# citiususc/veryfasttree

Hardware: AMD Instinct MI355X
Metric: profile-ops/sec (higher is better)
Workload: dtype f32; 1 GPU; c4_1M_x200_nt_tophits; n_seqs=1000000, n_pos=200, active_nodes=750000, top_k=2000

## Files before the change

### veryfasttree_amd/csrc/vft_api.hip

```cpp
#include <hip/hip_runtime.h>
#include <csignal>
#include <unistd.h>

#include <cmath>
#include <cstdarg>
#include <cstdio>
#include <cstdlib>
#include <cstring>
#include <new>
#include <algorithm>
#include <utility>
#include <vector>
#include <chrono>

#include "../../include/vft_hip.h"
#include "vft_owned.h"
#include "vft_staging.h"
#define VFT_PAIR_STAGE_CAP 2048
#include "vft_kernels_ml.h"

VFT_ML_HEAVY_INSTANCES(extern)
#include "vft_kernels_ml_long.h"
VFT_ML_LONG_INSTANCES(extern)
#include "vft_kernels_nj.h"
// ... 1915 lines not shown
    if (ids) {
        if (n <= 0) return VFT_OK;
        if (nActive > c->maxStamp) c->maxStamp = nActive;
        if (n == 1) {
            if (ids[0] < 0 || ids[0] >= c->maxnode) return fail(c, VFT_ERR_INVALID, "vft_out_distances: bad node");
            SweepArgs s{};
            s.nActive = nActive;
            s.totdiam = totdiam;
            s.force = 1;
            VFT_DISPATCH(c, launch((k_out_distance_one<REAL, NC>), dim3(1), dim3(VFT_WG), pw_lds_bytes(c) / c->pwWaves, c->stream,
                                   arena<REAL>(c), ids[0], s));
            LAUNCHCHK(c);
            return VFT_OK;
        }
        Stage st;
        if (int r = st.open(c, (size_t) n * 8, VFT_SMALL_BYTES)) return r;
        VFTCHK(st.put(0, ids, (size_t) n * 8));
        if (int r = launch_out_distances(c, st.dev<const int64_t>(0), n, nActive, 0, totdiam, true)) return r;
        return st.finish();
    }
    return launch_out_distances(c, nullptr, 0, nActive, 0, totdiam, true);
}

static void kernel_event(vft_ctx *c) {
    if (!c->timeKernels) return;
    if (c->kevUsed == c->kev.size()) {
        hipEvent_t e;
        if (hipEventCreate(&e) != hipSuccess) return;
        c->kev.push_back(e);
    }
    hipEventRecord(c->kev[c->kevUsed++], c->stream);
}

static int64_t slot_nodes(const vft_ctx *c, int slot) { return (c->d.nTiles + (slot ? 4 : 0)) * VFT_TILE; }

static int ensure_slots(vft_ctx *c, int count) {
    if (count > VFT_MAX_SLOTS) return fail(c, VFT_ERR_INVALID, "more than %d sweep slots", VFT_MAX_SLOTS);
    c->slots.reserve(VFT_MAX_SLOTS);
    const size_t rs = c->rs;
    bool added = false;
    while ((int) c->slots.size() < count) {
        const int slot = (int) c->slots.size();
        const size_t N = (size_t) slot_nodes(c, slot);
        c->slots.emplace_back();
        vft_ctx::SweepSlotHost &h = c->slots.back();
        const int r = own_group(c, [&]() -> int {
            void **reals[] = {&h.swDist, &h.swWeight, &h.swCrit};
            for (void **p: reals) OWNCHK(own_dev(c, p, N * rs, 0));
            const size_t nPartCap = (size_t) cdiv((int64_t) N, VFT_WG);
            OWNCHK(own_dev(c, &h.partMin, nPartCap * 8));
            OWNCHK(own_dev(c, &h.partMax, nPartCap * 8));
            OWNCHK(own_dev(c, &h.sel, sizeof(SelectState), 0));
            OWNCHK(own_dev(c, &h.slices, (size_t) VFT_NBINS * 4, 0));
            OWNCHK(own_dev(c, &h.candKey, (size_t) VFT_CAND_CAP * 8, 0));
            OWNCHK(own_dev(c, &h.candId, (size_t) VFT_CAND_CAP * 4, 0));
            const size_t resB = sizeof(SelectHeader) + (size_t) c->hitsCap * sizeof(vft_hit_f64);
            OWNCHK(own_dev(c, &h.dRes, resB));
            OWNCHK(own_host(c, &h.hRes, &h.hResDev, resB, sizeof(SelectHeader)));
            if (slot > 0 && c->cfg.n_codes == 4) {
                const size_t nPosPad = (size_t) c->d.nChunk * VFT_CHUNK;
                OWNCHK(own_dev(c, &h.qW, nPosPad * rs));
                OWNCHK(own_dev(c, &h.qF, nPosPad * 4 * rs));
                OWNCHK(own_dev(c, &h.qC, nPosPad));
                OWNCHK(own_dev(c, &h.qEnc, (size_t) c->d.nChunk * sizeof(uint4)));
                OWNCHK(own_dev(c, &h.qTab, nPosPad * 5 * sizeof(double2)));
            }
            return VFT_OK;
        });
        if (r) {
            c->slots.pop_back();
            return r;
        }
        added = true;
    }
    if (added) HIPCHK(c, hipDeviceSynchronize());
    return VFT_OK;
}

static int wait_headers(vft_ctx *c, int s0, int count, unsigned long long seq) {
    if (c->faultNoFlag) {
        seq += 1ull << 40;
        c->faultNoFlag = false;
    }
    auto raised = [&]() {
        for (int s = s0; s < s0 + count; s++)
            if ((unsigned long long) __atomic_load_n(&((const SelectHeader *) c->slots[(size_t) s].hRes)->pad2, __ATOMIC_ACQUIRE) != seq) return false;
        return true;
    };
    std::chrono::steady_clock::time_point t0;
    for (long spins = 0;; spins++) {
        if (raised()) return VFT_OK;
        if (spins == 200000) t0 = std::chrono::steady_clock::now();
        if (spins >= 200000 && (spins & 0xFFFF) == 0) {
            const hipError_t e = hipStreamQuery(c->stream);
            if (e == hipSuccess) {
                if (raised()) return VFT_OK;
                return fail(c, VFT_ERR_TIMEOUT, "the stream has drained but a selection never published its result");
            }
            if (e != hipErrorNotReady) return fail(c, VFT_ERR_HIP, "stream error while waiting: %s", hipGetErrorString(e));
            if (std::chrono::duration<double>(std::chrono::steady_clock::now() - t0).count() > c->waitLimitS)
                return fail(c, VFT_ERR_TIMEOUT, "no selection result after %.0f s (the stream is still busy)", c->waitLimitS);
        }
    }
}

template <typename REAL, typename HIT>
static int run_select(vft_ctx *c, int K, const int64_t *queries, int64_t lo, int64_t hi, int32_t k) {
    std::vector<SelSlot> hs((size_t) K);
    for (int s = 0; s < K; s++) {
        const vft_ctx::SweepSlotHost &h = c->slots[(size_t) s];
        SelSlot &d = hs[(size_t) s];
        d.crit = h.swCrit;
        d.dist = h.swDist;
        d.weight = h.swWeight;
        d.partMin = h.partMin;
        d.partMax = h.partMax;
        d.sel = h.sel;
        d.slices = h.slices;
        d.candKey = h.candKey;
        d.candId = h.candId;
        d.hits = h.dRes + sizeof(SelectHeader);
        d.hdr = (SelectHeader *) h.dRes;
        d.hostHdr = (SelectHeader *) h.hResDev;
        d.hostHits = h.hResDev + sizeof(SelectHeader);
        d.query = queries[s];
        d.nPart = h.nPart;
        d.pad = 0;
    }
    Stage st;
    if (int r = st.open(c, hs.size() * sizeof(SelSlot), Stage::RING_ONLY)) return r;
    st.put(0, hs.data(), hs.size() * sizeof(SelSlot));
    const SelSlot *slots = st.dev<const SelSlot>(0);
    auto round = [&](const SelSlot *sl, unsigned ny, int first, int s0) -> int {
        const unsigned long long seq = ++c->signalSeq;
        launch((k_select_hist<REAL>), dim3(VFT_SEL_WGS, ny), dim3(VFT_WG), 0, c->stream, sl, lo, hi, first);
        launch((k_select_collect<REAL>), dim3(VFT_SEL_WGS, ny), dim3(VFT_WG), 0, c->stream, sl, lo, hi, (unsigned int) k);
        launch((k_select_rank<REAL, HIT>), dim3(VFT_CAND_CAP * VFT_RANK_LANES / VFT_WG, ny), dim3(VFT_WG), 0, c->stream, sl, k, lo, hi, (long long) seq);
        LAUNCHCHK(c);
        return wait_headers(c, s0, (int) ny, seq);
    };
    if (int r = round(slots, (unsigned) K, 1, 0)) return r;
    for (int s = 0; s < K; s++) {
        const SelectHeader *h = (const SelectHeader *) c->slots[(size_t) s].hRes;
        for (int level = 0; h->overflow; level++) {
            if (level == VFT_MAX_LEVEL)
                return fail(c, VFT_ERR_STATE, "top-k select: more than %d hits tied at the k-th criterion", VFT_CAND_CAP);
            launch(k_select_refine, dim3(1, 1), dim3(1), 0, c->stream, slots + s);
            if (int r = round(slots + s, 1u, 0, s)) return r;
        }
    }
    return VFT_OK;
}

static int sweep_one(vft_ctx *c, int slot, int64_t query, int64_t nActive, int64_t nDiffAllow, double totdiam, bool staged = false) {
    if (int r = flush_pending(c)) return r;
    const int64_t lo = c->shardLo, hi = c->shardHi < c->maxnode ? c->shardHi : c->maxnode;
    if (c->maxStamp - nActive > nDiffAllow)
        if (int r = launch_out_distances(c, nullptr, 0, nActive, nDiffAllow, totdiam, false)) return r;
    if ((int64_t) c->hNOut[query] - nActive > nDiffAllow) {
        if (nActive > c->maxStamp) c->maxStamp = nActive;
        SweepArgs s{};
        s.nActive = nActive;
        s.nDiffAllow = nDiffAllow;
        s.totdiam = totdiam;
        s.force = 0;
        VFT_DISPATCH(c, launch((k_out_distance_one<REAL, NC>), dim3(1), dim3(VFT_WG), pw_lds_bytes(c) / c->pwWaves, c->stream,
                               arena<REAL>(c), query, s));
        LAUNCHCHK(c);
    }
    SweepArgs s{};
    s.query = query;
    s.lo = lo;
    s.hi = hi;
    s.nActive = nActive;
    s.nDiffAllow = nDiffAllow;
    s.totdiam = totdiam;
    s.queryIsLeaf = query < c->d.nSeqs ? 1 : 0;
#ifdef VFT_ABLATE
    if (const char *dbg = getenv("VFT_SWEEP_ABLATE")) s.pad = atoi(dbg);
#endif
    const int64_t span = hi > lo ? hi - lo : 0;
    const bool ntPath = c->cfg.n_codes == 4 && !c->hasDm;
    const unsigned grid = ntPath ? sweep_nt_grid(c, s, !s.queryIsLeaf) : cdiv(span > 0 ? span : 1, VFT_WG);
    c->slots[(size_t) slot].nPart = (int) grid;
    const int64_t nPosPad = (int64_t) c->d.nChunk * VFT_CHUNK;
    if (c->cfg.n_codes == 4 && !c->hasDm) {
        if (c->cfg.precision == 4) {
            const QueryBuf<float> Q = staged ? qbuf_slot<float>(c, slot) : qbuf<float>(c, 0);
            if (!staged) launch((k_extract_query<float, 4>), dim3(cdiv(nPosPad, 256)), dim3(256), 0, c->stream, arena<float>(c), query, Q);
            if (s.queryIsLeaf) launch_sweep_nt<float, MODE_CRIT_LEAFQ>(c, s, grid, Q, true, slot);
            else launch_sweep_nt<float, MODE_CRIT>(c, s, grid, Q, true, slot);
        } else {
            const QueryBuf<double> Q = staged ? qbuf_slot<double>(c, slot) : qbuf<double>(c, 0);
            if (!staged) launch((k_extract_query<double, 4>), dim3(cdiv(nPosPad, 256)), dim3(256), 0, c->stream, arena<double>(c), query, Q);
            if (s.queryIsLeaf) launch_sweep_nt<double, MODE_CRIT_LEAFQ>(c, s, grid, Q, true, slot);
            else launch_sweep_nt<double, MODE_CRIT>(c, s, grid, Q, true, slot);
        }
    } else {
        kernel_event(c);
        if (c->cfg.n_codes == 20 && c->hasDm && c->aaLds && span > 0) {
            const unsigned g = c->cfg.precision == 4 ? launch_sweep_aa<float, MODE_CRIT>(c, s, 0, slot) : launch_sweep_aa<double, MODE_CRIT>(c, s, 0, slot);
            c->slots[(size_t) slot].nPart = (int) g;
        } else if (span <= 32768) {
            const unsigned wgrid = (unsigned) std::min<int64_t>(cdiv(span > 0 ? span : 1, c->pwWaves), 256 * 16);
            c->slots[(size_t) slot].nPart = (int) wgrid;
            VFT_DISPATCH(c, (launch((k_sweep_wave<REAL, NC>), dim3(wgrid), dim3(64 * c->pwWaves), pw_lds_bytes(c), c->stream,
                                    arena<REAL>(c), s, sweepout<REAL>(c, slot))));
        } else {
            VFT_DISPATCH(c, (launch((k_sweep_generic<REAL, NC>), dim3(grid), dim3(VFT_WG), 0, c->stream,
                                    arena<REAL>(c), s, sweepout<REAL>(c, slot))));
        }
        kernel_event(c);
        kernel_event(c);
    }
    LAUNCHCHK(c);
    return VFT_OK;
}

template <typename REAL, int S>
static int sweep_group(vft_ctx *c, bool leafSeeds, const int *slotOf, const int64_t *queries, int64_t nActive, int64_t nDiffAllow, double totdiam, const void *mq, const void *lq) {
    SweepArgs s{};
    s.query = queries[slotOf[0]];
    s.lo = c->shardLo;
    s.hi = c->shardHi < c->maxnode ? c->shardHi : c->maxnode;
    s.nActive = nActive;
    s.nDiffAllow = nDiffAllow;
    s.totdiam = totdiam;
    s.queryIsLeaf = leafSeeds ? 1 : 0;
    const unsigned grid = sweep_nt_grid(c, s, !leafSeeds);
    MultiLeafQ<REAL, S> M;
    for (int q = 0; q < S; q++) {
        M.Q[q] = qbuf_slot<REAL>(c, slotOf[q]);
        M.O[q] = sweepout<REAL>(c, slotOf[q]);
        M.query[q] = queries[slotOf[q]];
        c->slots[(size_t) slotOf[q]].nPart = (int) grid;
    }
    M.mq = (const REAL *) mq;
    M.lq = (const uint32_t *) lq;
    kernel_event(c);
    if (grid && leafSeeds) launch((k_sweep_nt_leafq_multi<REAL, S>), dim3(grid), dim3(VFT_WG), 0, c->stream, arena<REAL>(c), M, s);
    if (grid && !leafSeeds) launch((k_sweep_nt_profq_multi<REAL, S>), dim3(grid), dim3(VFT_WG), 0, c->stream, arena<REAL>(c), M, s);
    kernel_event(c);
    kernel_event(c);
    if (c->timeKernels) c->kevSweeps += S - 1;
    LAUNCHCHK(c);
    return VFT_OK;
}

static bool mixed_sweep_fits(vft_ctx *c) {
    SweepArgs s{};
    s.lo = c->shardLo;
    s.hi = c->shardHi < c->maxnode ? c->shardHi : c->maxnode;
    const unsigned grid = sweep_nt_grid(c, s, true);
    if (!s.nLeafWG || grid == (unsigned) s.nLeafWG || s.hi <= s.leafEnd) return false;
    if (c->rs != 4) return false;
    const int64_t N = slot_nodes(c, 1);
    return (int64_t) cdiv(s.leafEnd - s.lo, VFT_WG) + (int64_t) (grid - (unsigned) s.nLeafWG) <= (int64_t) cdiv(N, VFT_WG);
}

template <typename REAL>
static int sweep_mixed(vft_ctx *c, const int *leafPos, const int *profPos, const int64_t *queries, int64_t nActive, int64_t nDiffAllow, double totdiam, const void *mq, const void *lq) {
    constexpr int S = 4;
    MixedArgs<REAL, S, S> a;
    memset((void *) &a, 0, sizeof(a));
    a.A = arena<REAL>(c);
    SweepArgs &s = a.s;
    s.query = queries[profPos[0]];
    s.lo = c->shardLo;
    s.hi = c->shardHi < c->maxnode ? c->shardHi : c->maxnode;
    s.nActive = nActive;
    s.nDiffAllow = nDiffAllow;
    s.totdiam = totdiam;
    s.queryIsLeaf = 0;
    const unsigned gridP = sweep_nt_grid(c, s, true);
    a.nInt = (int32_t) (gridP - (unsigned) s.nLeafWG);
    a.nLeafHeavy = (int32_t) cdiv(s.leafEnd - s.lo, VFT_WG);
    for (int q = 0; q < S; q++) {
        a.M.L.Q[q] = qbuf_slot<REAL>(c, leafPos[q]);
        a.M.L.O[q] = sweepout<REAL>(c, leafPos[q]);
        a.M.L.query[q] = queries[leafPos[q]];
        c->slots[(size_t) leafPos[q]].nPart = a.nLeafHeavy + a.nInt;
        a.M.P.Q[q] = qbuf_slot<REAL>(c, profPos[q]);
        a.M.P.O[q] = sweepout<REAL>(c, profPos[q]);
        a.M.P.query[q] = queries[profPos[q]];
        c->slots[(size_t) profPos[q]].nPart = (int) gridP;
    }
    a.M.L.mq = nullptr;
    a.M.L.lq = (const uint32_t *) lq;
    a.M.P.mq = (const REAL *) mq;
    a.M.P.lq = nullptr;
    kernel_event(c);
    launch((k_sweep_nt_mixed_multi<REAL, S, S>), dim3((unsigned) (a.nInt + a.nLeafHeavy + s.nLeafWG)), dim3(VFT_WG), 0, c->stream, a);
    kernel_event(c);
    kernel_event(c);
    if (c->timeKernels) c->kevSweeps += 2 * S - 1;
    LAUNCHCHK(c);
    return VFT_OK;
}

static int no_slot(vft_ctx *c) { return fail(c, VFT_ERR_STATE, "the context has no sweep buffers (vft_create failed)"); }

static int sweep_args_ok(vft_ctx *c, int64_t query, int64_t nActive, int32_t k) {
    if (c->slots.empty()) return no_slot(c);
    if (!c->leavesUp) return fail(c, VFT_ERR_STATE, "vft_sweep before vft_upload_leaves");
    if (query < 0 || query >= c->maxnode || nActive < 3 || k < 0 || k > c->hitsCap)
        return fail(c, VFT_ERR_INVALID, "vft_sweep: bad arguments (query %lld, nActive %lld, k %d)", (long long) query,
// ... 2045 lines not shown
```

### veryfasttree_amd/csrc/vft_kernels_nj.h

```cpp
#pragma once
#include "vft_device.h"

#define VFT_WG 256

template <typename REAL>
struct QueryBuf {
    REAL *w;
    uint8_t *code;
    REAL *f;
    uint4 *enc;
    double2 *tab;
};

template <typename REAL>
__device__ __forceinline__ void vft_query_tab(const QueryBuf<REAL> &q, int64_t p, REAL wq, const REAL *f) {
#pragma unroll
    for (int c = 0; c < 5; c++) {
        double2 v = make_double2(0.0, 0.0);
        if (c < 4 && wq > 0) {
            const double wgt = (double) wq;
            const double piece = 1.0 - (double) f[c < 4 ? c : 0];
            v = make_double2(wgt * piece, wgt);
        }
        q.tab[p * 5 + c] = v;
// ... 1896 lines not shown
        const REAL dd = A.diameter[i] + A.diameter[j];
        d = d - dd;
    }
    dist[t] = d;
}

#define VFT_PB_A 8
template <typename REAL, int NC>
__global__ __launch_bounds__(VFT_WG) void k_pairs_block_tiled(Arena<REAL> A, const int64_t *idsA, int64_t nA, const int64_t *idsB,
                                                              int64_t nB, REAL *dist) {
    extern __shared__ __attribute__((aligned(16))) double pbLds[];
    const int64_t nPos = A.d.nPos;
    REAL *sF = (REAL *) pbLds;
    REAL *sWt = sF + (int64_t) VFT_PB_A * nPos * NC;
    int32_t *sCode = (int32_t *) (sWt + (int64_t) VFT_PB_A * nPos);
    const int64_t a0 = (int64_t) blockIdx.y * VFT_PB_A;
    for (int64_t e = threadIdx.x; e < (int64_t) VFT_PB_A * nPos; e += VFT_WG) {
        const int64_t a = e / nPos, p = e % nPos;
        const int64_t id = a0 + a < nA ? idsA[a0 + a] : -1;
        Col<REAL, NC> c;
        c.w = 0;
        c.code = VFT_NOCODE_;
        c.vec = false;
#pragma unroll
        for (int k = 0; k < NC; k++) c.f[k] = 0;
        if (id >= 0) vft_load_col_ml<REAL, NC>(A, id, p, c);
        sWt[e] = c.w;
        sCode[e] = c.code | (c.vec ? 256 : 0);
#pragma unroll
        for (int k = 0; k < NC; k++) sF[e * NC + k] = c.vec ? c.f[k] : (REAL) 0;
    }
    __syncthreads();
    const int64_t b = (int64_t) blockIdx.x * VFT_WG + threadIdx.x;
    const int64_t jb = b < nB ? idsB[b] : -1;
    if (jb < 0) return;
    double top[VFT_PB_A], den[VFT_PB_A];
#pragma unroll
    for (int a = 0; a < VFT_PB_A; a++) top[a] = den[a] = 0.0;
    for (int64_t p = 0; p < nPos; p++) {
        Col<REAL, NC> cb;
        vft_load_col_ml<REAL, NC>(A, jb, p, cb);
        if (!(cb.w > 0)) continue;
#pragma unroll
        for (int a = 0; a < VFT_PB_A; a++) {
            const int64_t e = (int64_t) a * nPos + p;
            Col<REAL, NC> ca;
            ca.w = sWt[e];
            if (!(ca.w > 0)) continue;
            const int32_t cc = sCode[e];
            ca.code = cc & 255;
            ca.vec = (cc & 256) != 0;
#pragma unroll
            for (int k = 0; k < NC; k++) ca.f[k] = sF[e * NC + k];
            const REAL ww = ca.w * cb.w;
            const double wgt = (double) ww;
            den[a] += wgt;
            top[a] += wgt * vft_piece<REAL, NC>(A, ca, cb, nullptr);
        }
    }
#pragma unroll
    for (int a = 0; a < VFT_PB_A; a++) {
        if (a0 + a >= nA) break;
        const int64_t i = idsA[a0 + a];
        if (i < 0 || i == jb) continue;
        REAL d = (REAL) (den[a] > 0 ? top[a] / den[a] : 1.0);
        if (!(i < A.d.nSeqs && jb < A.d.nSeqs)) {
            const REAL dd = A.diameter[i] + A.diameter[jb];
            d = d - dd;
        }
        dist[(a0 + a) * nB + b] = d;
    }
}

template <typename REAL, int NC, bool WGPAIR>
__global__ __launch_bounds__(VFT_WG) void k_refresh_list(Arena<REAL> A, const int64_t *ids, int64_t n, int64_t nForced, SweepArgs s) {
    extern __shared__ __attribute__((aligned(16))) double pwLds[];
    const int64_t t = WGPAIR ? (int64_t) blockIdx.x : (int64_t) blockIdx.x * VFT_PW_WAVES + (threadIdx.x >> 6);
    if (t >= n) return;
    const int64_t v = ids[t];
    if (t < nForced ? (int64_t) A.nOutActive[v] == s.nActive : !((int64_t) A.nOutActive[v] - s.nActive > s.nDiffAllow)) return;
    REAL d, w;
    if (WGPAIR) vft_pair_block<REAL, NC>(A, v, -1, true, pwLds, pwLds + A.d.nPosPad, d, w);
    else vft_pair_wave<REAL, NC>(A, v, -1, true, vft_pw_lds(pwLds, A.d.nPosPad, 0), vft_pw_lds(pwLds, A.d.nPosPad, 1), d, w);
    if ((WGPAIR ? threadIdx.x : (threadIdx.x & 63)) != 0) return;
    const REAL od = vft_out_distance<REAL>(d, w, s.nActive, A.selfweight[v], A.selfdist[v], A.diameter[v], s.totdiam);
    A.outDist[v] = od;
    A.mOutDist[v] = od;
    A.mNOut[v] = (int32_t) s.nActive;
    A.nOutActive[v] = (int32_t) s.nActive;
}

#define VFT_LB_A 16
template <typename REAL>
__global__ __launch_bounds__(VFT_WG) void k_leaf_block(Arena<REAL> A, const int64_t *idsA, int64_t nA, const int64_t *idsB,
                                                       int64_t nB, SweepArgs s, REAL *dist, REAL *weight, REAL *crit) {
    const int lane = threadIdx.x & 63, wave = __builtin_amdgcn_readfirstlane((int) (threadIdx.x >> 6));
    const int64_t tb = (int64_t) blockIdx.x * 64 + lane;
    const int64_t a0 = (int64_t) blockIdx.y * 64 + (int64_t) wave * VFT_LB_A;
    if (a0 >= nA) return;
    const int64_t b = tb < nB ? idsB[tb] : -1;
    const bool bOk = b >= 0 && b < A.d.nSeqs;
    const uint4 *bT = A.leafT + vft_leaf_idx(A.d, bOk ? b >> 6 : 0, 0, (int) (bOk ? b & 63 : 0));
    int64_t aId[VFT_LB_A];
    const uint4 *aT[VFT_LB_A];
#pragma unroll
    for (int u = 0; u < VFT_LB_A; u++) {
        int64_t a = a0 + u < nA ? idsA[a0 + u] : -1;
        if (a < 0 || a >= A.d.nSeqs) a = -1;
        aId[u] = a;
        aT[u] = A.leafT + vft_leaf_idx(A.d, a >= 0 ? a >> 6 : 0, 0, (int) (a >= 0 ? a & 63 : 0));
    }
    int nUse[VFT_LB_A], nSame[VFT_LB_A];
#pragma unroll
    for (int u = 0; u < VFT_LB_A; u++) nUse[u] = nSame[u] = 0;
    const int nChunk = A.d.nChunk;
    for (int c = 0; c < nChunk; c++) {
        const uint4 vb = bT[(int64_t) c * VFT_TILE];
#pragma unroll
        for (int u = 0; u < VFT_LB_A; u++) {
            typedef const __attribute__((address_space(4))) vft_u4_t *sp_t;
            const vft_u4_t q = *(sp_t) (aT[u] + (int64_t) c * VFT_TILE);
            uint4 va;
            va.x = q.x; va.y = q.y; va.z = q.z; va.w = q.w;
            vft_seq_counts(va, vb, nUse[u], nSame[u]);
        }
    }
    if (tb >= nB) return;
    const REAL outB = bOk ? A.outDist[b] : (REAL) 0;
    const int64_t nOutB = bOk ? A.nOutActive[b] : s.nActive;
#pragma unroll
    for (int u = 0; u < VFT_LB_A; u++) {
        if (a0 + u >= nA) break;
        const int64_t a = aId[u];
        REAL d = (REAL) 1e20, w = 0, cr = (REAL) 1e20;
        if (a >= 0 && bOk) {
            w = (REAL) (double) nUse[u];
            d = (REAL) (nUse[u] > 0 ? (double) (nUse[u] - nSame[u]) / (double) nUse[u] : 1.0);
            cr = vft_criterion<REAL>(d, A.outDist[a], A.nOutActive[a], outB, nOutB, s.nActive);
        }
        const int64_t o = (a0 + u) * nB + tb;
        dist[o] = d;
        weight[o] = w;
        crit[o] = cr;
    }
}

#define VFT_NBINS 1024
#define VFT_DIGIT_BITS 10
#define VFT_VK_FRAC_BITS 40
#define VFT_MAX_LEVEL 4
#define VFT_SEL_WGS 128
#define VFT_CAND_CAP 8192

struct SelectState {
    double lo, scale;
    unsigned long long prefix;
    unsigned int level;
    unsigned int threshBin;
    unsigned int nCand;
    unsigned int overflow;
    unsigned int nBelow;
    unsigned int nThresh;
    unsigned int nIn;
    unsigned int rankDone;
};

struct SelectHeader;
struct SelSlot {
    const void *crit, *dist, *weight;
    const void *partMin, *partMax;
    SelectState *sel;
    unsigned int *slices;
    uint64_t *candKey;
    int32_t *candId;
    void *hits;
    SelectHeader *hdr, *hostHdr;
    void *hostHits;
    int64_t query;
    int32_t nPart, pad;
};

__device__ __forceinline__ unsigned long long vft_vk(double x, double lo, double scale) {
    const double y = (x - lo) * scale;
    const double top = 1125899906842623.0;
    return y <= 0.0 ? 0ull : (y >= top ? (unsigned long long) top : (unsigned long long) y);
}
__device__ __forceinline__ unsigned int vft_level_shift(unsigned int level) {
    return (unsigned int) (VFT_VK_FRAC_BITS - VFT_DIGIT_BITS * (int) level);
}

__global__ void k_select_refine(const SelSlot *slots) {
    SelectState *S = slots[blockIdx.y].sel;
    S->nIn += S->nBelow;
    S->prefix = (S->prefix << VFT_DIGIT_BITS) | S->threshBin;
    S->level += 1;
    S->nCand = 0;
    S->overflow = 0;
    S->rankDone = 0;
}

template <typename REAL>
__global__ __launch_bounds__(VFT_WG) void k_select_hist(const SelSlot *slots, int64_t lo, int64_t hi, int first) {
    const SelSlot &sl = slots[blockIdx.y];
    const REAL *crit = (const REAL *) sl.crit;
    SelectState *S = sl.sel;
    unsigned int *slices = sl.slices;
    __shared__ unsigned int lh4[4][VFT_NBINS];
    unsigned int *lh = lh4[threadIdx.x & 3];
    __shared__ double smin[VFT_WG / 64], smax[VFT_WG / 64];
    for (int t = threadIdx.x; t < 4 * VFT_NBINS; t += VFT_WG) lh4[0][t] = 0;
    double vlo, scale;
    unsigned long long prefix;
    unsigned int level;
    if (first) {
        const REAL *partMin = (const REAL *) sl.partMin, *partMax = (const REAL *) sl.partMax;
        double cmin = 1e30, cmax = -1e30;
        for (int t = threadIdx.x; t < sl.nPart; t += VFT_WG) {
            const double a = (double) partMin[t], b = (double) partMax[t];
            cmin = a < cmin ? a : cmin;
            cmax = b > cmax ? b : cmax;
        }
#pragma unroll
        for (int off = 32; off > 0; off >>= 1) {
            const double a = __shfl_xor(cmin, off, 64), b = __shfl_xor(cmax, off, 64);
            cmin = a < cmin ? a : cmin;
            cmax = b > cmax ? b : cmax;
        }
        if ((threadIdx.x & 63) == 0) {
            smin[threadIdx.x >> 6] = cmin;
            smax[threadIdx.x >> 6] = cmax;
        }
        __syncthreads();
        cmin = smin[0];
        cmax = smax[0];
#pragma unroll
        for (int w = 1; w < VFT_WG / 64; w++) {
            cmin = smin[w] < cmin ? smin[w] : cmin;
            cmax = smax[w] > cmax ? smax[w] : cmax;
        }
        const double span = cmax > cmin ? cmax - cmin : 1.0;
        vlo = cmin;
        scale = 1023.9990234375 * 1099511627776.0 / span;
        prefix = 0;
        level = 0;
        if (blockIdx.x == 0 && threadIdx.x == 0) {
            S->lo = vlo;
            S->scale = scale;
            S->prefix = 0;
            S->level = 0;
            S->nCand = 0;
            S->overflow = 0;
            S->nIn = 0;
            S->rankDone = 0;
        }
    } else {
        __syncthreads();
        vlo = S->lo;
        scale = S->scale;
        prefix = S->prefix;
        level = S->level;
    }
    const unsigned int shift = vft_level_shift(level);
    const int64_t stride = (int64_t) gridDim.x * VFT_WG;
    int64_t j = lo + (int64_t) blockIdx.x * VFT_WG + threadIdx.x;
    for (; j + 3 * stride < hi; j += 4 * stride) {
        REAL c[4];
#pragma unroll
        for (int u = 0; u < 4; u++) c[u] = crit[j + u * stride];
#pragma unroll
        for (int u = 0; u < 4; u++) {
            if (c[u] < (REAL) 1e20) {
                const unsigned long long vk = vft_vk((double) c[u], vlo, scale);
                if ((vk >> (shift + VFT_DIGIT_BITS)) == prefix) atomicAdd(&lh[(vk >> shift) & (VFT_NBINS - 1)], 1u);
            }
        }
    }
    for (; j < hi; j += stride) {
        const REAL c = crit[j];
        if (c < (REAL) 1e20) {
            const unsigned long long vk = vft_vk((double) c, vlo, scale);
            if ((vk >> (shift + VFT_DIGIT_BITS)) == prefix) atomicAdd(&lh[(vk >> shift) & (VFT_NBINS - 1)], 1u);
        }
    }
    __syncthreads();
    for (int t = threadIdx.x; t < VFT_NBINS; t += VFT_WG) {
        const unsigned int v = lh4[0][t] + lh4[1][t] + lh4[2][t] + lh4[3][t];
        if (v) atomicAdd(&slices[t], v);
    }
}

template <typename REAL>
__global__ __launch_bounds__(VFT_WG) void k_select_collect(const SelSlot *slots, int64_t lo, int64_t hi, unsigned int k) {
    const SelSlot &sl = slots[blockIdx.y];
    const REAL *crit = (const REAL *) sl.crit;
    SelectState *S = sl.sel;
    uint64_t *candKey = sl.candKey;
    int32_t *candId = sl.candId;
    __shared__ unsigned int lcount, lbase;
    __shared__ uint64_t lkey[VFT_CAND_CAP / 8];
    __shared__ int32_t lid[VFT_CAND_CAP / 8];
    if (threadIdx.x == 0) lcount = 0;
    __shared__ unsigned int wsum[VFT_WG / 64], sTb, sBelow, sThresh;
    unsigned int tb;
    {
        constexpr int PER = VFT_NBINS / VFT_WG;
        const unsigned int *gh = sl.slices;
        const int lane = threadIdx.x & 63, wave = threadIdx.x >> 6;
        unsigned int v[PER], mine = 0;
#pragma unroll
        for (int u = 0; u < PER; u++) {
            v[u] = gh[threadIdx.x * PER + u];
            mine += v[u];
        }
        unsigned int incl = mine;
#pragma unroll
        for (int off = 1; off < 64; off <<= 1) {
            const unsigned int o = __shfl_up(incl, off, 64);
            if (lane >= off) incl += o;
        }
        if (lane == 63) wsum[wave] = incl;
        if (threadIdx.x == 0) {
            sTb = VFT_NBINS;
            sBelow = 0;
            sThresh = 0;
        }
        __syncthreads();
        unsigned int before = incl - mine, total = 0;
#pragma unroll
        for (int w = 0; w < VFT_WG / 64; w++) {
            if (w < wave) before += wsum[w];
            total += wsum[w];
        }
        unsigned int need = k > S->nIn ? k - S->nIn : 0;
        if (need > total) need = total;
        if (need > 0 && before < need && before + mine >= need) {
            unsigned int b = before;
#pragma unroll
            for (int u = 0; u < PER; u++) {
                if (b < need && b + v[u] >= need) {
                    sTb = (unsigned int) (threadIdx.x * PER + u);
                    sBelow = b;
                    sThresh = v[u];
                }
                b += v[u];
            }
        }
        __syncthreads();
        tb = sTb;
        if (blockIdx.x == 0 && threadIdx.x == 0) {
            S->threshBin = tb;
            S->nBelow = sBelow;
            S->nThresh = sThresh;
        }
    }
    const double vlo = S->lo, scale = S->scale;
    const unsigned long long prefix = S->prefix;
    const unsigned int shift = vft_level_shift(S->level);
    const int64_t stride = (int64_t) gridDim.x * VFT_WG;
    auto take = [&](int64_t j, REAL c) {
        if (!(c < (REAL) 1e20)) return;
        const unsigned long long vk = vft_vk((double) c, vlo, scale);
        const unsigned long long up = vk >> (shift + VFT_DIGIT_BITS);
        if (up < prefix || (up == prefix && tb < VFT_NBINS && ((vk >> shift) & (VFT_NBINS - 1)) <= tb)) {
            const unsigned int slot = atomicAdd(&lcount, 1u);
            if (slot < VFT_CAND_CAP / 8) {
                lkey[slot] = sizeof(REAL) == 4 ? (uint64_t) vft_order_f32((float) c) : vft_order_f64((double) c);
                lid[slot] = (int32_t) j;
            }
        }
    };
    int64_t j = lo + (int64_t) blockIdx.x * VFT_WG + threadIdx.x;
    for (; j + 3 * stride < hi; j += 4 * stride) {
        REAL c[4];
#pragma unroll
        for (int u = 0; u < 4; u++) c[u] = crit[j + u * stride];
#pragma unroll
        for (int u = 0; u < 4; u++) take(j + u * stride, c[u]);
    }
    for (; j < hi; j += stride) take(j, crit[j]);
    __syncthreads();
    const unsigned int n = lcount;
    if (n > VFT_CAND_CAP / 8) {
        if (threadIdx.x == 0) S->overflow = 1;
        return;
    }
    if (threadIdx.x == 0) lbase = n ? atomicAdd(&S->nCand, n) : 0;
    __syncthreads();
    const unsigned int base = lbase;
    if (base + n > VFT_CAND_CAP) {
        if (threadIdx.x == 0) S->overflow = 1;
        return;
    }
    for (unsigned int t = threadIdx.x; t < n; t += VFT_WG) {
        candKey[base + t] = lkey[t];
        candId[base + t] = lid[t];
    }
}

struct SelectHeader {
    unsigned int nCand, overflow, shift, pad;
    long long bestJ;
    long long pad2;
};

template <typename HIT>
__device__ __forceinline__ void vft_hit_publish(HIT *dst, const HIT &h) {
    static_assert(sizeof(HIT) % 8 == 0, "hit records are whole 8-byte words");
    unsigned long long w[sizeof(HIT) / 8];
    __builtin_memcpy(w, &h, sizeof(HIT));
#pragma unroll
    for (unsigned int t = 0; t < sizeof(HIT) / 8; t++)
        __hip_atomic_store((unsigned long long *) dst + t, w[t], __ATOMIC_RELAXED, __HIP_MEMORY_SCOPE_AGENT);
}
template <typename HIT>
__device__ __forceinline__ HIT vft_hit_fetch(const HIT *src) {
    unsigned long long w[sizeof(HIT) / 8];
#pragma unroll
    for (unsigned int t = 0; t < sizeof(HIT) / 8; t++)
        w[t] = __hip_atomic_load((const unsigned long long *) src + t, __ATOMIC_RELAXED, __HIP_MEMORY_SCOPE_AGENT);
    HIT h;
    __builtin_memcpy(&h, w, sizeof(HIT));
    return h;
}

#define VFT_RANK_TILE 2048
#define VFT_RANK_LANES 16
template <typename REAL, typename HIT>
__global__ __launch_bounds__(VFT_WG) void k_select_rank(const SelSlot *slots, int32_t k, int64_t lo, int64_t hi, long long seq) {
    const SelSlot &sl = slots[blockIdx.y];
    SelectState *S = sl.sel;
    const uint64_t *candKey = sl.candKey;
    const int32_t *candId = sl.candId;
    const REAL *dist = (const REAL *) sl.dist, *weight = (const REAL *) sl.weight, *crit = (const REAL *) sl.crit;
    HIT *hits = (HIT *) sl.hits;
    HIT *hostHits = (HIT *) sl.hostHits;
    __shared__ uint64_t sk[VFT_RANK_TILE];
    __shared__ int32_t si[VFT_RANK_TILE];
    const unsigned int n = S->overflow ? 0u : (S->nCand < VFT_CAND_CAP ? S->nCand : VFT_CAND_CAP);
    const unsigned int perWg = VFT_WG / VFT_RANK_LANES;
    const unsigned int span = n > (unsigned int) k ? n : (unsigned int) k;
    if (blockIdx.x * perWg >= span) return;
    const unsigned int cand = blockIdx.x * perWg + threadIdx.x / VFT_RANK_LANES;
    const unsigned int sub = threadIdx.x % VFT_RANK_LANES;
    const bool mine = cand < n;
    const uint64_t myKey = mine ? candKey[cand] : 0;
    const int32_t myId = mine ? candId[cand] : 0;
    unsigned int rank = 0;
    for (unsigned int base = 0; base < n; base += VFT_RANK_TILE) {
        __syncthreads();
        for (unsigned int u = threadIdx.x; u < VFT_RANK_TILE; u += VFT_WG) {
            sk[u] = base + u < n ? candKey[base + u] : ~0ull;
            si[u] = base + u < n ? candId[base + u] : -1;
        }
        __syncthreads();
        const unsigned int lim = n - base < VFT_RANK_TILE ? n - base : VFT_RANK_TILE;
        if (mine) {
#pragma unroll 8
            for (unsigned int u = sub; u < lim; u += VFT_RANK_LANES) {
                const uint64_t ku = sk[u];
                const int32_t iu = si[u];
                rank += (ku < myKey || (ku == myKey && iu > myId)) ? 1u : 0u;
            }
        }
    }
#pragma unroll
    for (int off = VFT_RANK_LANES / 2; off > 0; off >>= 1) rank += __shfl_xor(rank, off, VFT_RANK_LANES);
    if (sub == 0) {
        if (mine && rank < (unsigned int) k) {
            HIT h;
            h.j = myId;
            h.dist = dist[myId];
            h.weight = weight[myId];
            h.criterion = crit[myId];
            vft_hit_publish<HIT>(hits + rank, h);
        }
        if (cand >= n && cand < (unsigned int) k) {
            HIT h;
            h.j = -1;
            h.dist = (REAL) 1e20;
            h.weight = 0;
            h.criterion = (REAL) 1e20;
            vft_hit_publish<HIT>(hits + cand, h);
        }
    }
    __shared__ unsigned int sLast;
    asm volatile("s_waitcnt vmcnt(0)" ::: "memory");
    __syncthreads();
    if (threadIdx.x == 0) {
        const unsigned int active = (span + perWg - 1) / perWg;
        sLast = __hip_atomic_fetch_add(&S->rankDone, 1u, __ATOMIC_RELAXED, __HIP_MEMORY_SCOPE_AGENT) == active - 1 ? 1u : 0u;
    }
    __syncthreads();
    if (!sLast) return;
    const int64_t query = sl.query;
    SelectHeader *hdr = sl.hdr, *hostHdr = sl.hostHdr;
    __shared__ long long sBest;
    __shared__ REAL sCrit;
    __shared__ int sTruncatedTie;
    for (int t = threadIdx.x; t < VFT_NBINS; t += VFT_WG) sl.slices[t] = 0;
    for (int t0 = 0; t0 < k; t0 += 8 * VFT_WG) {
        HIT tmp[8];
#pragma unroll
        for (int u = 0; u < 8; u++) {
            const int t = t0 + u * VFT_WG + (int) threadIdx.x;
            tmp[u] = vft_hit_fetch<HIT>(hits + (t < k ? t : 0));
        }
#pragma unroll
        for (int u = 0; u < 8; u++) {
            const int t = t0 + u * VFT_WG + (int) threadIdx.x;
            if (t < k) hostHits[t] = tmp[u];
        }
    }
    if (threadIdx.x == 0) {
        const unsigned int nn = n < (unsigned int) k ? n : (unsigned int) k;
        long long best = -1;
        REAL bc = (REAL) 1e20;
        unsigned int t = 0;
        for (; t < nn; t++) {
            const HIT h = vft_hit_fetch<HIT>(hits + t);
            const long long j = (long long) h.j;
            if (j == query || j < 0) continue;
            const REAL c = h.criterion;
            if (best < 0) {
                if (!(c < (REAL) 1e20)) break;
                best = j;
                bc = c;
            } else if (c == bc) {
                if (j < best) best = j;
            } else {
                break;
            }
        }
        sBest = best;
        sCrit = bc;
        sTruncatedTie = (best >= 0 && t == nn && nn == (unsigned int) k) ? 1 : 0;
    }
    __syncthreads();
    if (sTruncatedTie) {
        const REAL bc = sCrit;
        long long mineJ = sBest;
        for (int64_t j = lo + threadIdx.x; j < hi; j += VFT_WG)
            if (j != query && crit[j] == bc && j < mineJ) mineJ = j;
        atomicMin((unsigned long long *) &sBest, (unsigned long long) mineJ);
        __syncthreads();
    }
    __threadfence_system();
    asm volatile("s_waitcnt vmcnt(0)" ::: "memory");
    __syncthreads();
    if (threadIdx.x != 0) return;
    SelectHeader h;
    h.nCand = S->nCand;
    h.overflow = S->overflow;
    h.shift = S->level;
    h.pad = 0;
    h.bestJ = sBest;
    h.pad2 = 0;
    *hdr = h;
    hostHdr->nCand = h.nCand;
    hostHdr->overflow = h.overflow;
    hostHdr->shift = h.shift;
    hostHdr->pad = 0;
    hostHdr->bestJ = h.bestJ;
    __hip_atomic_store(&hostHdr->pad2, seq, __ATOMIC_RELEASE, __HIP_MEMORY_SCOPE_SYSTEM);
}

template <typename REAL, typename HIT>
__global__ __launch_bounds__(VFT_WG) void k_merge_hits(const HIT *all, int32_t n, int32_t k, HIT *out, HIT *hostOut,
                                                       int32_t nSeeds) {
    __shared__ REAL sc[VFT_RANK_TILE];
    __shared__ long long sj[VFT_RANK_TILE];
    const unsigned int seed = blockIdx.y;
    auto rec = [&](unsigned int u) -> const HIT & {
        return all[((size_t) (u / (unsigned int) k) * (unsigned int) nSeeds + seed) * (unsigned int) k + u % (unsigned int) k];
    };
    out += (size_t) seed * k;
    hostOut += (size_t) seed * k;
    const unsigned int perWg = VFT_WG / VFT_RANK_LANES;
    const unsigned int cand = blockIdx.x * perWg + threadIdx.x / VFT_RANK_LANES;
    const unsigned int sub = threadIdx.x % VFT_RANK_LANES;
    const bool mine = cand < (unsigned int) n;
    const REAL myC = mine ? rec(cand).criterion : (REAL) 0;
    const long long myJ = mine ? (long long) rec(cand).j : -1;
    unsigned int rank = 0;
    for (unsigned int base = 0; base < (unsigned int) n; base += VFT_RANK_TILE) {
        __syncthreads();
        for (unsigned int u = threadIdx.x; u < VFT_RANK_TILE; u += VFT_WG) {
            const bool in = base + u < (unsigned int) n;
            sc[u] = in ? rec(base + u).criterion : (REAL) 0;
            sj[u] = in ? (long long) rec(base + u).j : -1;
        }
        __syncthreads();
        const unsigned int lim = (unsigned int) n - base < VFT_RANK_TILE ? (unsigned int) n - base : VFT_RANK_TILE;
        if (mine && myJ >= 0) {
#pragma unroll 8
            for (unsigned int u = sub; u < lim; u += VFT_RANK_LANES) {
                const long long ju = sj[u];
                const REAL cu = sc[u];
                rank += (ju >= 0 && (cu < myC || (cu == myC && ju > myJ))) ? 1u : 0u;
            }
        }
    }
#pragma unroll
    for (int off = VFT_RANK_LANES / 2; off > 0; off >>= 1) rank += __shfl_xor(rank, off, VFT_RANK_LANES);
    if (sub != 0 || !mine || myJ < 0) return;
    if (rank < (unsigned int) k) {
        out[rank] = rec(cand);
        hostOut[rank] = rec(cand);
    }
}

template <typename REAL, typename HIT>
__global__ void k_fill_empty_hits(HIT *out, HIT *hostOut, int32_t k) {
    const int t = blockIdx.x * blockDim.x + threadIdx.x;
    if (t >= k) return;
    HIT h;
    h.j = -1;
    h.dist = (REAL) 1e20;
    h.weight = 0;
    h.criterion = (REAL) 1e20;
    out[t] = h;
    hostOut[t] = h;
}
```

Measured before the change: 15.43 billion profile-ops/s.

## Vectorize and prefetch top-k select scans, pack rank keys, parallelize best-hit scan

After: 15.99 billion profile-ops/s (median of 6 runs). 1.04x the previous value.

```diff
diff --git a/veryfasttree_amd/csrc/vft_api.hip b/veryfasttree_amd/csrc/vft_api.hip
--- a/veryfasttree_amd/csrc/vft_api.hip
+++ b/veryfasttree_amd/csrc/vft_api.hip
@@ -2091,6 +2091,17 @@
     return VFT_OK;
 }
 
+#ifdef VFT_SELECT_PHASES
+extern "C" int vft_debug_select_phases(vft_ctx *c, unsigned long long *out, int64_t nOut) {
+    if (nOut != (int64_t) VFT_SELPH_ROWS * VFT_SELPH_SEEDS * VFT_SELPH_MARKS) return fail(c, VFT_ERR_INVALID, "vft_debug_select_phases: %d x %d x %d words", VFT_SELPH_ROWS, VFT_SELPH_SEEDS, VFT_SELPH_MARKS);
+    HIPCHK(c, hipStreamSynchronize(c->stream));
+    HIPCHK(c, hipMemcpyFromSymbol(out, HIP_SYMBOL(vft_selph), sizeof(vft_selph)));
+    static const unsigned long long zero[VFT_SELPH_ROWS][VFT_SELPH_SEEDS][VFT_SELPH_MARKS] = {};
+    HIPCHK(c, hipMemcpyToSymbol(HIP_SYMBOL(vft_selph), zero, sizeof(zero)));
+    return VFT_OK;
+}
+#endif
+
 static int sweep_one(vft_ctx *c, int slot, int64_t query, int64_t nActive, int64_t nDiffAllow, double totdiam, bool staged = false) {
     if (int r = flush_pending(c)) return r;
     const int64_t lo = c->shardLo, hi = c->shardHi < c->maxnode ? c->shardHi : c->maxnode;
diff --git a/veryfasttree_amd/csrc/vft_kernels_nj.h b/veryfasttree_amd/csrc/vft_kernels_nj.h
--- a/veryfasttree_amd/csrc/vft_kernels_nj.h
+++ b/veryfasttree_amd/csrc/vft_kernels_nj.h
@@ -2072,6 +2072,24 @@
 #define VFT_SEL_WGS 128
 #define VFT_CAND_CAP 8192
 
+#ifdef VFT_SELECT_PHASES
+#define VFT_SELPH_ROWS 4
+#define VFT_SELPH_SEEDS 16
+#define VFT_SELPH_MARKS 8
+__device__ unsigned long long vft_selph[VFT_SELPH_ROWS][VFT_SELPH_SEEDS][VFT_SELPH_MARKS];
+#define VFT_SELPH(row, mark)                                                                                           \
+    do {                                                                                                               \
+        if (threadIdx.x == 0 && (blockIdx.x == 0 || (row) == 3) && blockIdx.y < VFT_SELPH_SEEDS)                       \
+            vft_selph[row][blockIdx.y][mark] = wall_clock64();                                                         \
+    } while (0)
+#define VFT_SELPH_USE(x) asm volatile("" ::"v"(x))
+#define VFT_SELPH_DRAIN() asm volatile("s_waitcnt vmcnt(0)" ::: "memory")
+#else
+#define VFT_SELPH(row, mark) ((void) 0)
+#define VFT_SELPH_USE(x) ((void) 0)
+#define VFT_SELPH_DRAIN() ((void) 0)
+#endif
+
 struct SelectState {
     double lo, scale;
     unsigned long long prefix;
@@ -2119,26 +2137,116 @@
     S->rankDone = 0;
 }
 
+#define VFT_SEL_BATCH 10
+#define VFT_GLOBAL __attribute__((address_space(1)))
 template <typename REAL>
-__global__ __launch_bounds__(VFT_WG) void k_select_hist(const SelSlot *slots, int64_t lo, int64_t hi, int first) {
+struct SelVec {
+    static constexpr int N = 16 / (int) sizeof(REAL);
+    typedef REAL type __attribute__((ext_vector_type(16 / sizeof(REAL))));
+};
+template <typename REAL>
+struct SelSpan {
+    static constexpr int N = SelVec<REAL>::N;
+    typedef typename SelVec<REAL>::type V;
+    const VFT_GLOBAL REAL *crit;
+    const VFT_GLOBAL V *vp;
+    const VFT_GLOBAL V *spare;
+    int64_t lo, hi, first, nVec, stride, v0;
+    __device__ __forceinline__ SelSpan(const REAL *crit_, int64_t lo_, int64_t hi_, const void *spare_)
+        : crit((const VFT_GLOBAL REAL *) crit_), spare((const VFT_GLOBAL V *) spare_), lo(lo_), hi(hi_ > lo_ ? hi_ : lo_) {
+        const int64_t head = (N - (lo & (N - 1))) & (N - 1);
+        first = lo + head < hi ? lo + head : hi;
+        nVec = (hi - first) / N;
+        vp = (const VFT_GLOBAL V *) (crit + first);
+        stride = (int64_t) gridDim.x * VFT_WG;
+        v0 = (int64_t) blockIdx.x * VFT_WG + threadIdx.x;
+    }
+    __device__ __forceinline__ void load(int64_t vb, V (&c)[VFT_SEL_BATCH]) const {
+#pragma unroll
+        for (int u = 0; u < VFT_SEL_BATCH; u++) {
+            const int64_t v = vb + v0 + (int64_t) u * stride;
+            c[u] = *(v < nVec ? vp + v : spare);
+        }
+    }
+    template <typename F>
+    __device__ __forceinline__ void consume(int64_t vb, V (&c)[VFT_SEL_BATCH], F f) const {
+        int64_t v = vb + v0;
+#pragma unroll 1
+        for (int u = 0; u < VFT_SEL_BATCH; u++, v += stride) {
+            V x = c[0];
+#pragma unroll
+            for (int w = 0; w + 1 < VFT_SEL_BATCH; w++) c[w] = c[w + 1];
+#pragma unroll
+            for (int e = 0; e < N; e++) x[e] = v < nVec ? x[e] : (REAL) 1e20;
+            f(first + v * N, x);
+        }
+    }
+    __device__ __forceinline__ REAL load_edge(int64_t &j) const {
+        const int64_t t = threadIdx.x;
+        const int64_t e = t < N - 1 ? lo + t : first + nVec * N + (t - (N - 1));
+        const bool ok = blockIdx.x == gridDim.x - 1 && t < 2 * (N - 1) && (t < N - 1 ? e < first : e < hi);
+        const REAL x = *(ok ? crit + e : (const VFT_GLOBAL REAL *) spare);
+        j = ok ? e : -1;
+        return ok ? x : (REAL) 1e20;
+    }
+};
+
+#define VFT_SEL_PART_BATCH 5
+template <typename REAL>
+__global__ __launch_bounds__(VFT_WG, 4) void k_select_hist(const SelSlot *slots, int64_t lo, int64_t hi, int first) {
     const SelSlot &sl = slots[blockIdx.y];
     const REAL *crit = (const REAL *) sl.crit;
     SelectState *S = sl.sel;
     unsigned int *slices = sl.slices;
+    typedef typename SelVec<REAL>::type V;
+    constexpr int N = SelVec<REAL>::N;
+    const SelSpan<REAL> sp(crit, lo, hi, sl.slices);
     __shared__ unsigned int lh4[4][VFT_NBINS];
     unsigned int *lh = lh4[threadIdx.x & 3];
     __shared__ double smin[VFT_WG / 64], smax[VFT_WG / 64];
+    VFT_SELPH(0, 0);
+    const VFT_GLOBAL REAL *partMin = (const VFT_GLOBAL REAL *) sl.partMin, *partMax = (const VFT_GLOBAL REAL *) sl.partMax;
+    const int nPart = first ? sl.nPart : 0, nPartVec = nPart / N;
+    V pa[VFT_SEL_PART_BATCH], pb[VFT_SEL_PART_BATCH];
+    auto load_parts = [&](int p0) {
+#pragma unroll
+        for (int u = 0; u < VFT_SEL_PART_BATCH; u++) {
+            const int p = p0 + u * VFT_WG + (int) threadIdx.x;
+            pa[u] = *(p < nPartVec ? (const VFT_GLOBAL V *) partMin + p : sp.spare);
+            pb[u] = *(p < nPartVec ? (const VFT_GLOBAL V *) partMax + p : sp.spare);
+        }
+    };
+    load_parts(0);
+    const int pt = nPartVec * N + (int) threadIdx.x < nPart ? nPartVec * N + (int) threadIdx.x : 0;
+    const REAL pta = partMin[pt], ptb = partMax[pt];
+    V c[VFT_SEL_BATCH];
+    sp.load(0, c);
+    int64_t je;
+    const REAL ce = sp.load_edge(je);
     for (int t = threadIdx.x; t < 4 * VFT_NBINS; t += VFT_WG) lh4[0][t] = 0;
     double vlo, scale;
     unsigned long long prefix;
     unsigned int level;
     if (first) {
-        const REAL *partMin = (const REAL *) sl.partMin, *partMax = (const REAL *) sl.partMax;
         double cmin = 1e30, cmax = -1e30;
-        for (int t = threadIdx.x; t < sl.nPart; t += VFT_WG) {
-            const double a = (double) partMin[t], b = (double) partMax[t];
-            cmin = a < cmin ? a : cmin;
-            cmax = b > cmax ? b : cmax;
+        auto fold_parts = [&](int p0) {
+#pragma unroll
+            for (int u = 0; u < VFT_SEL_PART_BATCH; u++) {
+                const bool in = p0 + u * VFT_WG + (int) threadIdx.x < nPartVec;
+#pragma unroll
+                for (int e = 0; e < N; e++) {
+                    const double a = (double) pa[u][e], b = (double) pb[u][e];
+                    cmin = in && a < cmin ? a : cmin;
+                    cmax = in && b > cmax ? b : cmax;
+                }
+            }
+        };
+        fold_parts(0);
+        cmin = (double) pta < cmin ? (double) pta : cmin;
+        cmax = (double) ptb > cmax ? (double) ptb : cmax;
+        for (int p0 = VFT_SEL_PART_BATCH * VFT_WG; p0 < nPartVec; p0 += VFT_SEL_PART_BATCH * VFT_WG) {
+            load_parts(p0);
+            fold_parts(p0);
         }
 #pragma unroll
         for (int off = 32; off > 0; off >>= 1) {
@@ -2181,36 +2289,36 @@
         level = S->level;
     }
     const unsigned int shift = vft_level_shift(level);
-    const int64_t stride = (int64_t) gridDim.x * VFT_WG;
-    int64_t j = lo + (int64_t) blockIdx.x * VFT_WG + threadIdx.x;
-    for (; j + 3 * stride < hi; j += 4 * stride) {
-        REAL c[4];
-#pragma unroll
-        for (int u = 0; u < 4; u++) c[u] = crit[j + u * stride];
-#pragma unroll
-        for (int u = 0; u < 4; u++) {
-            if (c[u] < (REAL) 1e20) {
-                const unsigned long long vk = vft_vk((double) c[u], vlo, scale);
-                if ((vk >> (shift + VFT_DIGIT_BITS)) == prefix) atomicAdd(&lh[(vk >> shift) & (VFT_NBINS - 1)], 1u);
-            }
-        }
-    }
-    for (; j < hi; j += stride) {
-        const REAL c = crit[j];
-        if (c < (REAL) 1e20) {
-            const unsigned long long vk = vft_vk((double) c, vlo, scale);
+    VFT_SELPH_USE(scale);
+    VFT_SELPH(0, 1);
+    auto bin = [&](REAL x) {
+        if (x < (REAL) 1e20) {
+            const unsigned long long vk = vft_vk((double) x, vlo, scale);
             if ((vk >> (shift + VFT_DIGIT_BITS)) == prefix) atomicAdd(&lh[(vk >> shift) & (VFT_NBINS - 1)], 1u);
         }
+    };
+    bin(ce);
+    for (int64_t vb = 0;;) {
+        sp.consume(vb, c, [&](int64_t, const V &x) {
+#pragma unroll
+            for (int e = 0; e < N; e++) bin(x[e]);
+        });
+        vb += VFT_SEL_BATCH * sp.stride;
+        if (vb >= sp.nVec) break;
+        sp.load(vb, c);
     }
     __syncthreads();
+    VFT_SELPH(0, 2);
     for (int t = threadIdx.x; t < VFT_NBINS; t += VFT_WG) {
         const unsigned int v = lh4[0][t] + lh4[1][t] + lh4[2][t] + lh4[3][t];
         if (v) atomicAdd(&slices[t], v);
     }
+    VFT_SELPH_DRAIN();
+    VFT_SELPH(0, 3);
 }
 
 template <typename REAL>
-__global__ __launch_bounds__(VFT_WG) void k_select_collect(const SelSlot *slots, int64_t lo, int64_t hi, unsigned int k) {
+__global__ __launch_bounds__(VFT_WG, 4) void k_select_collect(const SelSlot *slots, int64_t lo, int64_t hi, unsigned int k) {
     const SelSlot &sl = slots[blockIdx.y];
     const REAL *crit = (const REAL *) sl.crit;
     SelectState *S = sl.sel;
@@ -2220,18 +2328,31 @@
     __shared__ uint64_t lkey[VFT_CAND_CAP / 8];
     __shared__ int32_t lid[VFT_CAND_CAP / 8];
     if (threadIdx.x == 0) lcount = 0;
+    VFT_SELPH(1, 0);
+    typedef typename SelVec<REAL>::type V;
+    constexpr int N = SelVec<REAL>::N;
+    const SelSpan<REAL> sp(crit, lo, hi, sl.slices);
+    const VFT_GLOBAL SelectState *Sg = (const VFT_GLOBAL SelectState *) S;
+    const unsigned int nIn = Sg->nIn;
+    const double vlo = Sg->lo, scale = Sg->scale;
+    const unsigned long long prefix = Sg->prefix;
+    const unsigned int shift = vft_level_shift(Sg->level);
+    static_assert(VFT_NBINS / VFT_WG == 4, "a thread's share of the histogram is one 16-byte vector");
+    typedef unsigned int u4_t __attribute__((ext_vector_type(4)));
+    const u4_t gh4 = ((const VFT_GLOBAL u4_t *) sl.slices)[threadIdx.x];
+    V c[VFT_SEL_BATCH];
+    sp.load(0, c);
+    int64_t je;
+    const REAL ce = sp.load_edge(je);
     __shared__ unsigned int wsum[VFT_WG / 64], sTb, sBelow, sThresh;
     unsigned int tb;
     {
         constexpr int PER = VFT_NBINS / VFT_WG;
-        const unsigned int *gh = sl.slices;
         const int lane = threadIdx.x & 63, wave = threadIdx.x >> 6;
-        unsigned int v[PER], mine = 0;
-#pragma unroll
-        for (int u = 0; u < PER; u++) {
-            v[u] = gh[threadIdx.x * PER + u];
-            mine += v[u];
-        }
+        const unsigned int v[PER] = {gh4.x, gh4.y, gh4.z, gh4.w};
+        unsigned int mine = 0;
+#pragma unroll
+        for (int u = 0; u < PER; u++) mine += v[u];
         unsigned int incl = mine;
 #pragma unroll
         for (int off = 1; off < 64; off <<= 1) {
@@ -2251,7 +2372,7 @@
             if (w < wave) before += wsum[w];
             total += wsum[w];
         }
-        unsigned int need = k > S->nIn ? k - S->nIn : 0;
+        unsigned int need = k > nIn ? k - nIn : 0;
         if (need > total) need = total;
         if (need > 0 && before < need && before + mine >= need) {
             unsigned int b = before;
@@ -2273,10 +2394,10 @@
             S->nThresh = sThresh;
         }
     }
-    const double vlo = S->lo, scale = S->scale;
-    const unsigned long long prefix = S->prefix;
-    const unsigned int shift = vft_level_shift(S->level);
-    const int64_t stride = (int64_t) gridDim.x * VFT_WG;
+    VFT_SELPH(1, 1);
+    VFT_SELPH_USE(scale);
+    VFT_SELPH_USE(shift);
+    VFT_SELPH(1, 2);
     auto take = [&](int64_t j, REAL c) {
         if (!(c < (REAL) 1e20)) return;
         const unsigned long long vk = vft_vk((double) c, vlo, scale);
@@ -2289,16 +2410,18 @@
             }
         }
     };
-    int64_t j = lo + (int64_t) blockIdx.x * VFT_WG + threadIdx.x;
-    for (; j + 3 * stride < hi; j += 4 * stride) {
-        REAL c[4];
-#pragma unroll
-        for (int u = 0; u < 4; u++) c[u] = crit[j + u * stride];
-#pragma unroll
-        for (int u = 0; u < 4; u++) take(j + u * stride, c[u]);
-    }
-    for (; j < hi; j += stride) take(j, crit[j]);
+    take(je, ce);
+    for (int64_t vb = 0;;) {
+        sp.consume(vb, c, [&](int64_t j, const V &x) {
+#pragma unroll
+            for (int e = 0; e < N; e++) take(j + e, x[e]);
+        });
+        vb += VFT_SEL_BATCH * sp.stride;
+        if (vb >= sp.nVec) break;
+        sp.load(vb, c);
+    }
     __syncthreads();
+    VFT_SELPH(1, 3);
     const unsigned int n = lcount;
     if (n > VFT_CAND_CAP / 8) {
         if (threadIdx.x == 0) S->overflow = 1;
@@ -2306,6 +2429,7 @@
     }
     if (threadIdx.x == 0) lbase = n ? atomicAdd(&S->nCand, n) : 0;
     __syncthreads();
+    VFT_SELPH(1, 4);
     const unsigned int base = lbase;
     if (base + n > VFT_CAND_CAP) {
         if (threadIdx.x == 0) S->overflow = 1;
@@ -2315,6 +2439,8 @@
         candKey[base + t] = lkey[t];
         candId[base + t] = lid[t];
     }
+    VFT_SELPH_DRAIN();
+    VFT_SELPH(1, 5);
 }
 
 struct SelectHeader {
@@ -2356,42 +2482,74 @@
     HIT *hostHits = (HIT *) sl.hostHits;
     __shared__ uint64_t sk[VFT_RANK_TILE];
     __shared__ int32_t si[VFT_RANK_TILE];
-    const unsigned int n = S->overflow ? 0u : (S->nCand < VFT_CAND_CAP ? S->nCand : VFT_CAND_CAP);
+    VFT_SELPH(2, 0);
+    static_assert(offsetof(SelectState, nCand) % 8 == 0 && offsetof(SelectState, overflow) == offsetof(SelectState, nCand) + 4,
+                  "nCand and overflow are read as one word");
     const unsigned int perWg = VFT_WG / VFT_RANK_LANES;
+    const unsigned int cand = blockIdx.x * perWg + threadIdx.x / VFT_RANK_LANES;
+    const unsigned int sub = threadIdx.x % VFT_RANK_LANES;
+    unsigned long long candOver;
+    __builtin_memcpy(&candOver, &S->nCand, 8);
+    const uint64_t key0 = cand < VFT_CAND_CAP ? candKey[cand] : 0;
+    const int32_t id0 = cand < VFT_CAND_CAP ? candId[cand] : 0;
+    const unsigned int nCand = (unsigned int) candOver, overflow = (unsigned int) (candOver >> 32);
+    const unsigned int n = overflow ? 0u : (nCand < VFT_CAND_CAP ? nCand : VFT_CAND_CAP);
     const unsigned int span = n > (unsigned int) k ? n : (unsigned int) k;
     if (blockIdx.x * perWg >= span) return;
-    const unsigned int cand = blockIdx.x * perWg + threadIdx.x / VFT_RANK_LANES;
-    const unsigned int sub = threadIdx.x % VFT_RANK_LANES;
+    VFT_SELPH(2, 1);
     const bool mine = cand < n;
-    const uint64_t myKey = mine ? candKey[cand] : 0;
-    const int32_t myId = mine ? candId[cand] : 0;
+    const uint64_t myKey = mine ? key0 : 0;
+    const int32_t myId = mine ? id0 : 0;
+    REAL myDist = 0, myWeight = 0, myCrit = 0;
+    if (mine && sub == 0) {
+        myDist = dist[myId];
+        myWeight = weight[myId];
+        myCrit = crit[myId];
+    }
+    constexpr bool PACKED = sizeof(REAL) == 4;
+    auto packed = [](uint64_t key, int32_t id) -> uint64_t { return (key << 32) | (uint64_t) (0xFFFFFFFFu - (uint32_t) id); };
+    const uint64_t myWord = packed(myKey, myId);
     unsigned int rank = 0;
     for (unsigned int base = 0; base < n; base += VFT_RANK_TILE) {
         __syncthreads();
         for (unsigned int u = threadIdx.x; u < VFT_RANK_TILE; u += VFT_WG) {
-            sk[u] = base + u < n ? candKey[base + u] : ~0ull;
-            si[u] = base + u < n ? candId[base + u] : -1;
+            const uint64_t ku = base + u < n ? candKey[base + u] : ~0ull;
+            const int32_t iu = base + u < n ? candId[base + u] : -1;
+            if (PACKED) {
+                sk[u] = base + u < n ? packed(ku, iu) : ~0ull;
+            } else {
+                sk[u] = ku;
+                si[u] = iu;
+            }
         }
         __syncthreads();
+        VFT_SELPH(2, 2);
         const unsigned int lim = n - base < VFT_RANK_TILE ? n - base : VFT_RANK_TILE;
         if (mine) {
+            if (PACKED) {
 #pragma unroll 8
-            for (unsigned int u = sub; u < lim; u += VFT_RANK_LANES) {
-                const uint64_t ku = sk[u];
-                const int32_t iu = si[u];
-                rank += (ku < myKey || (ku == myKey && iu > myId)) ? 1u : 0u;
+                for (unsigned int u = sub; u < lim; u += VFT_RANK_LANES) rank += sk[u] < myWord ? 1u : 0u;
+            } else {
+#pragma unroll 8
+                for (unsigned int u = sub; u < lim; u += VFT_RANK_LANES) {
+                    const uint64_t ku = sk[u];
+                    const int32_t iu = si[u];
+                    rank += (ku < myKey || (ku == myKey && iu > myId)) ? 1u : 0u;
+                }
             }
         }
     }
 #pragma unroll
     for (int off = VFT_RANK_LANES / 2; off > 0; off >>= 1) rank += __shfl_xor(rank, off, VFT_RANK_LANES);
+    VFT_SELPH_USE(rank);
+    VFT_SELPH(2, 3);
     if (sub == 0) {
         if (mine && rank < (unsigned int) k) {
             HIT h;
             h.j = myId;
-            h.dist = dist[myId];
-            h.weight = weight[myId];
-            h.criterion = crit[myId];
+            h.dist = myDist;
+            h.weight = myWeight;
+            h.criterion = myCrit;
             vft_hit_publish<HIT>(hits + rank, h);
         }
         if (cand >= n && cand < (unsigned int) k) {
@@ -2406,18 +2564,23 @@
     __shared__ unsigned int sLast;
     asm volatile("s_waitcnt vmcnt(0)" ::: "memory");
     __syncthreads();
+    VFT_SELPH(2, 4);
     if (threadIdx.x == 0) {
         const unsigned int active = (span + perWg - 1) / perWg;
         sLast = __hip_atomic_fetch_add(&S->rankDone, 1u, __ATOMIC_RELAXED, __HIP_MEMORY_SCOPE_AGENT) == active - 1 ? 1u : 0u;
     }
     __syncthreads();
+    VFT_SELPH(2, 5);
     if (!sLast) return;
+    VFT_SELPH(3, 0);
     const int64_t query = sl.query;
     SelectHeader *hdr = sl.hdr, *hostHdr = sl.hostHdr;
     __shared__ long long sBest;
     __shared__ REAL sCrit;
     __shared__ int sTruncatedTie;
     for (int t = threadIdx.x; t < VFT_NBINS; t += VFT_WG) sl.slices[t] = 0;
+    __shared__ long long sHeadJ[64];
+    __shared__ REAL sHeadC[64];
     for (int t0 = 0; t0 < k; t0 += 8 * VFT_WG) {
         HIT tmp[8];
 #pragma unroll
@@ -2425,13 +2588,56 @@
             const int t = t0 + u * VFT_WG + (int) threadIdx.x;
             tmp[u] = vft_hit_fetch<HIT>(hits + (t < k ? t : 0));
         }
+        if (t0 == 0 && threadIdx.x < 64) {
+            sHeadJ[threadIdx.x] = (long long) tmp[0].j;
+            sHeadC[threadIdx.x] = tmp[0].criterion;
+        }
 #pragma unroll
         for (int u = 0; u < 8; u++) {
             const int t = t0 + u * VFT_WG + (int) threadIdx.x;
             if (t < k) hostHits[t] = tmp[u];
         }
     }
-    if (threadIdx.x == 0) {
+    VFT_SELPH(3, 1);
+    bool serialScan = false;
+    if (threadIdx.x < 64) {
+        const unsigned int nn = n < (unsigned int) k ? n : (unsigned int) k;
+        const long long j = nn ? sHeadJ[threadIdx.x] : -1;
+        const REAL c = nn ? sHeadC[threadIdx.x] : (REAL) 1e20;
+        const bool counts = threadIdx.x < nn && !(j == query || j < 0);
+        const unsigned long long mCounts = __ballot(counts);
+        long long best = -1;
+        REAL bc = (REAL) 1e20;
+        int truncated = 0;
+        if (mCounts == 0) {
+            serialScan = nn > 64;
+        } else {
+            const REAL c0 = __shfl(c, __ffsll((long long) mCounts) - 1, 64);
+            if (c0 < (REAL) 1e20) {
+                const unsigned long long mEnd = __ballot(counts && !(c == c0));
+                if (mEnd == 0 && nn > 64) {
+                    serialScan = true;
+                } else {
+                    const unsigned int end = mEnd ? (unsigned int) __ffsll((long long) mEnd) - 1 : 64u;
+                    long long mj = counts && threadIdx.x < end ? j : 0x7fffffffffffffffll;
+#pragma unroll
+                    for (int off = 32; off > 0; off >>= 1) {
+                        const long long o = __shfl_xor(mj, off, 64);
+                        mj = o < mj ? o : mj;
+                    }
+                    best = mj;
+                    bc = c0;
+                    truncated = (mEnd == 0 && nn == (unsigned int) k) ? 1 : 0;
+                }
+            }
+        }
+        if (!serialScan && threadIdx.x == 0) {
+            sBest = best;
+            sCrit = bc;
+            sTruncatedTie = truncated;
+        }
+    }
+    if (serialScan && threadIdx.x == 0) {
         const unsigned int nn = n < (unsigned int) k ? n : (unsigned int) k;
         long long best = -1;
         REAL bc = (REAL) 1e20;
@@ -2456,6 +2662,7 @@
         sTruncatedTie = (best >= 0 && t == nn && nn == (unsigned int) k) ? 1 : 0;
     }
     __syncthreads();
+    VFT_SELPH(3, 2);
     if (sTruncatedTie) {
         const REAL bc = sCrit;
         long long mineJ = sBest;
@@ -2467,6 +2674,7 @@
     __threadfence_system();
     asm volatile("s_waitcnt vmcnt(0)" ::: "memory");
     __syncthreads();
+    VFT_SELPH(3, 3);
     if (threadIdx.x != 0) return;
     SelectHeader h;
     h.nCand = S->nCand;
@@ -2482,6 +2690,8 @@
     hostHdr->pad = 0;
     hostHdr->bestJ = h.bestJ;
     __hip_atomic_store(&hostHdr->pad2, seq, __ATOMIC_RELEASE, __HIP_MEMORY_SCOPE_SYSTEM);
+    VFT_SELPH_DRAIN();
+    VFT_SELPH(3, 4);
 }
 
 template <typename REAL, typename HIT>
```
